# nonl4331/raytracing-rust

Hardware: NVIDIA B200
Metric: Mrays/s (higher is better)
Workload: dtype f32

## Files before the change

### raytracing-rust_b200/csrc/wavefront.cu

```cuda
#include "ptb_internal.h"
#include "ptb_traverse.cuh"
#include "ptb_packet.cuh"
#include "ptb_camcand.cuh"

namespace ptb {

struct RenderParams {
  uint32_t width, height, npix;
  uint32_t row_begin;
  uint32_t tile_w, tile_h;
  uint32_t group;
  uint32_t dir_bins;
  uint32_t sample_offset;
  uint32_t method, max_depth, rr_threshold;
  uint32_t k0, k1;
};

struct Queues {
  uint32_t* live;
  float4* shadow;
  uint32_t* win_count;
  uint32_t* win_prefix;
  uint32_t* seg_total;
  uint8_t* bin;
// ... 204 lines not shown
      uint32_t x, y, sample;
      camera_pixel_sample(rp, first + i, x, y, sample);
      ray = make_ray(sc.cam_origin, camera_direction(sc, rp, x, y, sample));
      return;
    }
    slot = queue[i];
    float4 o, d;
    ldg256_rw(pool.ray + 4u * (size_t)slot, o, d);
    ray = make_ray(from4(o), from4(d));
  }
};
template <bool CAMERA>
struct TraceRetire {
  const PathPool& pool;
  const TraceFetch<CAMERA>& f;
  PTB_DEV void operator()(bool fin, const TraceResult& tr, const Ray& ray) {
    if (fin)
      stg256(pool.ray + 4u * (size_t)f.slot, make_float4(ray.o.x, ray.o.y, ray.o.z, tr.t),
             make_float4(ray.d.x, ray.d.y, ray.d.z, __uint_as_float(tr.ref)));
  }
};

#ifndef PTB_SHADE_MIN_BLOCKS
#define PTB_SHADE_MIN_BLOCKS 4
#endif
template <class TR, bool COUNT, bool CAMERA>
__global__ void __launch_bounds__(256, TR::kTraceMinBlocks)
k_trace(DevScene sc, PathPool pool, Queues q, WaveCounters* wc, RenderParams rp, unsigned long long first) {
  const uint32_t lane = threadIdx.x & 31u;
  uint32_t cnt_nodes = 0, cnt_prims = 0, cnt_rays = 0;
  TraceFetch<CAMERA> fetch{pool, q.live, 0u, sc, rp, first};
  TraceRetire<CAMERA> retire{pool, fetch};
  persistent_trace<TR, false, COUNT>(sc, wc->n_trace, &wc->trace_head, fetch, retire, cnt_nodes, cnt_prims, cnt_rays);
  if (COUNT) {
    for (int off = 16; off > 0; off >>= 1) {
      cnt_nodes += __shfl_xor_sync(0xffffffffu, cnt_nodes, off);
      cnt_prims += __shfl_xor_sync(0xffffffffu, cnt_prims, off);
      cnt_rays += __shfl_xor_sync(0xffffffffu, cnt_rays, off);
    }
    if (lane == 0 && cnt_rays) {
      atomicAdd(&wc->nodes_fetched, (unsigned long long)cnt_nodes);
      atomicAdd(&wc->prims_tested, (unsigned long long)cnt_prims);
      atomicAdd(&wc->rays_counted, (unsigned long long)cnt_rays);
    }
  }
}

#ifndef PTB_CAMERA_MIN_BLOCKS
#define PTB_CAMERA_MIN_BLOCKS 4
#endif
template <bool COUNT>
__global__ void __launch_bounds__(256, PTB_CAMERA_MIN_BLOCKS)
k_trace_camera(DevScene sc, PathPool pool, Queues q, WaveCounters* wc, RenderParams rp, unsigned long long first, CamCandList cl) {
  const uint32_t lane = threadIdx.x & 31u;
  const uint32_t n = wc->n_trace;
  uint32_t cnt_nodes = 0, cnt_prims = 0, cnt_rays = 0;
  for (;;) {
    uint32_t base = 0;
    if (lane == 0u) base = atomicAdd(&wc->trace_head, 32u);
    base = __shfl_sync(0xffffffffu, base, 0);
    if (base >= n) break;
    const uint32_t i = base + lane;
    const bool valid = i < n;
    Ray ray;
    uint32_t lin = 0;
    if (valid) {
      uint32_t x, y, sample;
      camera_pixel_sample(rp, first + i, x, y, sample);
      lin = (y - rp.row_begin) * rp.width + x;
      ray = make_ray(sc.cam_origin, camera_direction(sc, rp, x, y, sample));
      if (COUNT) ++cnt_rays;
    } else {
      ray = make_ray(sc.cam_origin, mk(0.0f, 0.0f, 1.0f));
    }
    float best_t;
    uint32_t best_ref;
    uint32_t cnt = kNone;
    if (cl.count) {
      const uint32_t lin0 = __shfl_sync(0xffffffffu, lin, 0);
      if (__all_sync(0xffffffffu, !valid || lin == lin0)) {
        lin = lin0;
        cnt = __ldg(cl.count + lin);
      }
    }
    if (cnt != kNone) cand_trace<COUNT>(sc, cl, lin, cnt, ray, valid, best_t, best_ref, cnt_prims);
    else packet_trace<COUNT>(sc, ray, valid, best_t, best_ref, cnt_nodes, cnt_prims);
    if (valid)
      stg256(pool.ray + 4u * (size_t)i, make_float4(ray.o.x, ray.o.y, ray.o.z, best_ref == kNone ? 0.0f : best_t),
             make_float4(ray.d.x, ray.d.y, ray.d.z, __uint_as_float(best_ref == kNone ? kNone : (best_ref & ~PTB_LEAF_BIT))));
  }
  if (COUNT) {
    for (int off = 16; off > 0; off >>= 1) {
      cnt_nodes += __shfl_xor_sync(0xffffffffu, cnt_nodes, off);
      cnt_prims += __shfl_xor_sync(0xffffffffu, cnt_prims, off);
      cnt_rays += __shfl_xor_sync(0xffffffffu, cnt_rays, off);
    }
    if (lane == 0 && cnt_rays) {
      atomicAdd(&wc->nodes_fetched, (unsigned long long)cnt_nodes);
      atomicAdd(&wc->prims_tested, (unsigned long long)cnt_prims);
      atomicAdd(&wc->rays_counted, (unsigned long long)cnt_rays);
    }
  }
}

struct Surface {
  HitRec h;
  uint32_t kind, tex, mat;
  float param;
  bool miss;
};

PTB_DEV float tr_d(float alpha, float cos_theta) {
  if (cos_theta <= 0.0f) return 0.0f;
  const float a_sq = alpha * alpha;
  const float tmp = cos_theta * cos_theta * (a_sq - 1.0f) + 1.0f;
  return a_sq / (kPi * tmp * tmp);
}
PTB_DEV float tr_g1(float alpha, v3 normal, v3 h, v3 v) {
  if (dot(v, h) / dot(v, normal) <= 0.0f) return 0.0f;
  const float c = dot(normal, v);
  const float cos_sq = c * c;
  const float alpha_sq = alpha * alpha;
  const float tmp = alpha_sq + (1.0f - alpha_sq) * cos_sq;
// ... 191 lines not shown
        shadow_is_sky = 1u;
      } else {
        const uint32_t lref = __ldg(sc.lights + li);
        l_wi = light_sample_dir(sc, lref, s.h.point, u32_to_unit(r.y), u32_to_unit(r.z));
        const Ray sray = make_ray_from_raw(so, l_wi);
        HitRec si;
        if (prim_hit(sc, sray, lref, si) && si.t > 0.0f) {
          const float pdf = light_pdf(sc, lref, s.h.point, l_wi, si.point, si.normal);
          if (pdf > 0.0f) {
            const uint32_t lmi = __ldg(sc.slot_mat + (lref & kSlotMask)) & 0x00FFFFFFu;
            const DevMaterial* lm = sc.materials + lmi;
            const v3 lpoint = offset_ray(si.point, si.normal, si.error, true);
            le = __ldg(&lm->param) * texture_colour<FULL>(sc, __ldg(&lm->tex), l_wi, lpoint);
            l_pdf = pdf * mult;
            tmax = si.t;
            exclude = lref & kSlotMask;
            usable = true;
          }
        }
      }
      if (usable) {
        const float mp = mat_scattering_pdf<FULL>(s, wo, l_wi);
        const float w = power_heuristic(l_pdf, mp);
        const v3 contrib = T * mat_eval<FULL>(sc, s, wo, l_wi) * w * le / l_pdf;
        const v3 sd = l_wi / mag(l_wi);
        sh_o = make_float4(so.x, so.y, so.z, tmax);
        sh_d = make_float4(sd.x, sd.y, sd.z, __uint_as_float(exclude));
        sh_c = make_float4(contrib.x, contrib.y, contrib.z, __uint_as_float(slot));
        shadow = true;
      }
    }
}

template <int METHOD, bool FULL>
PTB_DEV void shade_path(const DevScene& sc, const PathPool& pool, const RenderParams& rp, uint32_t slot, bool depth0,
                        unsigned long long camera_first, ShadeOut& o) {
  bool &alive = o.alive, &finished = o.finished, &shadow = o.shadow, &contributes = o.contributes;
  uint32_t &shadow_is_sky = o.shadow_is_sky, &fin_pixel = o.fin_pixel;
  float4 &sh_o = o.sh_o, &sh_d = o.sh_d, &sh_c = o.sh_c;
  v3& fin_L = o.fin_L;
  float4 ro, rd, th, ra;
  ldg256_rw(pool.ray + 4u * (size_t)slot, ro, rd);
  if (depth0) {
    uint32_t x, y, smp;
    camera_pixel_sample(rp, camera_first + slot, x, y, smp);
    th = make_float4(1.0f, 1.0f, 1.0f, __uint_as_float(y * rp.width + x));
    ra = make_float4(0.0f, 0.0f, 0.0f, __uint_as_float(smp << 9));
  } else {
    ldg256_rw(pool.col + 4u * (size_t)slot, th, ra);
  }
  const uint2 ht = make_uint2(__float_as_uint(ro.w), __float_as_uint(rd.w));
  const uint32_t pixel = __float_as_uint(th.w);
  const uint32_t df = __float_as_uint(ra.w);
  const uint32_t sample = df >> 9;
  uint32_t depth = df & 0xFFu;
  const bool prev_delta = (df & kFlagPrevDelta) != 0u;
  const Ray ray = make_ray(from4(ro), from4(rd));
  const v3 wo = ray.d;
  v3 T = from4(th), L = from4(ra);

  Surface s;
  s.miss = ht.y == kNone;
  if (s.miss) {
    s.h.t = 0.0f;
    s.h.point = s.h.error = s.h.normal = mk(0.0f, 0.0f, 0.0f);
    s.h.out = false;
    s.kind = PTB_MAT_EMIT;
    s.tex = sc.sky_tex;
    s.mat = 0u;
    s.param = 1.0f;
  } else {
    prim_hit(sc, ray, ht.y, s.h);
    const uint32_t mi = __ldg(sc.slot_mat + (ht.y & kSlotMask)) & 0x00FFFFFFu;
    const DevMaterial* m = sc.materials + mi;
    s.mat = mi;
    s.kind = __ldg(&m->kind);
    s.tex = __ldg(&m->tex);
    s.param = __ldg(&m->param);
  }
  const bool is_emit = s.kind == PTB_MAT_EMIT;
  bool depart = false;
  bool nan_check = true;

  if (METHOD == PTB_METHOD_NAIVE) {
    if (is_emit) {
      const v3 point = offset_ray(s.h.point, s.h.normal, s.h.error, true);
      const v3 emission = s.param * texture_colour<FULL>(sc, s.tex, wo, point);
      L = L + T * emission;
      finished = true;
    } else {
      depart = true;
    }
  } else {
    if (depth == 0u) {
      if (is_emit) {
        const v3 point = offset_ray(s.h.point, s.h.normal, s.h.error, true);
        L = L + s.param * texture_colour<FULL>(sc, s.tex, wo, point);
        finished = true;
        nan_check = false;
      } else {
        depth = 1u;
        depart = true;
      }
    } else {
      if (is_emit) {
        const v3 le = s.param * texture_colour<FULL>(sc, s.tex, wo, ray.o);
        if (!is_zero(le)) {
          const bool sky_samplable = (sc.sky_rx | sc.sky_ry) != 0u;
          const bool use_mis = s.miss ? sky_samplable : !prev_delta;
          if (use_mis) {
            const float divisor = (float)(sky_samplable ? sc.n_lights + 1u : sc.n_lights);
            const float4 pv = pool.prev[slot];
            const float l_pdf = s.miss ? sky_pdf(sc, wo) / divisor
                                       : light_pdf(sc, ht.y, from4(pv), wo, s.h.point, s.h.normal) / divisor;
            const float w = power_heuristic(pv.w, l_pdf);
            L = L + T * le * w;
          } else {
            L = L + T * le;
          }
        }
        finished = true;
      } else {
        bool survive = true;
        if (depth > rp.rr_threshold) {
          const float p = cmax3(T.x, T.y, T.z);
          const uint4 r = philox4x32_10(pixel, sample, (depth << 8) | RNG_RR, 0u, rp.k0, rp.k1);
          if (u32_to_unit(r.x) > p) survive = false;
          else T = T / p;
        }
        depth += 1u;
        if (survive && depth < rp.max_depth) depart = true;
        else finished = true;
      }
    }
  }

  if (depart) {
    float m_pdf = 0.0f;
    if (METHOD == PTB_METHOD_MIS) nee_sample<FULL>(sc, rp, s, wo, T, pixel, sample, depth, slot, o);
    const uint4 r = philox4x32_10(pixel, sample, (depth << 8) | RNG_SCATTER, 0u, rp.k0, rp.k1);
    v3 new_o, new_dir;
    bool delta = false;
    if (s.kind == PTB_MAT_LAMBERTIAN) {
      new_dir = lambertian_sample_dir(s.h.normal, u32_to_unit(r.x), u32_to_unit(r.y));
      new_o = offset_ray(s.h.point, s.h.normal, s.h.error, true);
    } else if (FULL && s.kind == PTB_MAT_TROWBRIDGE_REITZ) {
      new_dir = tr_sample(s.param, -wo, s.h.normal, u32_to_unit(r.x), u32_to_unit(r.y));
// ... 37 lines not shown
        else T = T / p;
      }
      depth += 1u;
      if (survive && depth < rp.max_depth) alive = true;
      else finished = true;
    } else {
      if (s.kind == PTB_MAT_LAMBERTIAN) {
        m_pdf = fmaxf(dot(nd, s.h.normal), 0.0f) / kPi;
        T = T * (col * s.param);
      } else if (is_tr) {
        m_pdf = mat_scattering_pdf<FULL>(s, wo, nd);
        T = T * col;
      } else {
        m_pdf = 0.0f;
        T = T * (col / 0.0f);
      }
      pool.prev[slot] = make_float4(s.h.point.x, s.h.point.y, s.h.point.z, m_pdf);
      alive = true;
    }
    if (alive) {
      stg256(pool.ray + 4u * (size_t)slot, make_float4(new_o.x, new_o.y, new_o.z, 0.0f),
             make_float4(nd.x, nd.y, nd.z, __uint_as_float(kNone)));
      stg256(pool.col + 4u * (size_t)slot, make_float4(T.x, T.y, T.z, th.w),
             make_float4(L.x, L.y, L.z, __uint_as_float((sample << 9) | (delta ? kFlagPrevDelta : 0u) | depth)));
      o.bin = rp.dir_bins ? direction_bin(nd) : 0u;
    }
  }
  if (finished) {
    contributes = !(nan_check && (contains_nan(L) || !any_finite(L)));
    fin_pixel = pixel;
    fin_L = L;
  }
}

template <int METHOD, bool FULL>
__global__ void __launch_bounds__(256, PTB_SHADE_MIN_BLOCKS + (METHOD == PTB_METHOD_MIS ? 1 : 0))
k_shade(DevScene sc, PathPool pool, Queues q, WaveCounters* wc, RenderParams rp, float* __restrict__ accum,
        unsigned long long camera_first, uint32_t sort_kinds) {
  const bool depth0 = camera_first != kNoCamera;
  const uint32_t lane = threadIdx.x & 31u;
  const uint32_t n_total = wc->n_trace;
  for (uint32_t base = blockIdx.x * blockDim.x; base < n_total; base += gridDim.x * blockDim.x) {
  const uint32_t i = base + threadIdx.x;
  bool active = i < n_total;

  uint32_t slot = 0;
  ShadeOut so;
  so.fin_L = mk(0.0f, 0.0f, 0.0f);

  if (active) slot = depth0 ? i : q.live[i];
  if (sort_kinds) {
    __shared__ uint32_t s_slot[256];
    __shared__ uint32_t s_cnt[(kNumKinds + 1) * 8];
    const uint32_t warp = threadIdx.x >> 5, n_warps = blockDim.x >> 5;
    uint32_t kind = (uint32_t)kNumKinds;
    if (active) {
      const uint32_t ref = __float_as_uint(pool.ray[4u * (size_t)slot + 1u].w);
      kind = ref == kNone ? 0u : 1u + (__ldg(sc.slot_mat + (ref & kSlotMask)) >> 24);
    }
    uint32_t rank = 0;
#pragma unroll
    for (uint32_t k = 0; k <= (uint32_t)kNumKinds; ++k) {
      const uint32_t m = __ballot_sync(0xffffffffu, kind == k);
      if (kind == k) rank = (uint32_t)__popc(m & ((1u << lane) - 1u));
      if (lane == 0u) s_cnt[k * 8u + warp] = (uint32_t)__popc(m);
    }
    __syncthreads();
    uint32_t pos = rank;
    for (uint32_t e = 0; e < kind * 8u + warp; ++e)
      if ((e & 7u) < n_warps) pos += s_cnt[e];
    s_slot[pos] = slot;
    __syncthreads();
    uint32_t n_here = 0;
    for (uint32_t e = 0; e < (uint32_t)kNumKinds * 8u; ++e)
      if ((e & 7u) < n_warps) n_here += s_cnt[e];
    active = threadIdx.x < n_here;
    slot = s_slot[threadIdx.x];
    __syncthreads();
  }
  if (active) shade_path<METHOD, FULL>(sc, pool, rp, slot, depth0, camera_first, so);
  finish_paths(accum, so.contributes, so.fin_pixel, so.fin_L);

  if (so.alive) q.bin[slot] = (uint8_t)so.bin;
  if (so.finished) q.bin[slot] = (uint8_t)kBinDead;
  const uint32_t window = slot / kWindow;
  const uint32_t peers = __match_any_sync(0xffffffffu, so.finished ? window : 0xffffffffu);
  if (so.finished && lane == (uint32_t)__ffs(peers) - 1u) atomicSub(&q.win_count[window], (uint32_t)__popc(peers));
  if (METHOD == PTB_METHOD_MIS) {
    const uint32_t m_sh = __ballot_sync(0xffffffffu, so.shadow), m_sky = __ballot_sync(0xffffffffu, so.shadow && so.shadow_is_sky);
    unsigned long long p2 = 0ull;
    if (lane == 0u && m_sh)
      p2 = atomicAdd(&wc->shadow_pair, ((unsigned long long)__popc(m_sky) << 32) | (unsigned long long)__popc(m_sh));
    p2 = __shfl_sync(0xffffffffu, p2, 0);
    if (so.shadow) {
      float4* e = q.shadow + 3u * (size_t)((uint32_t)p2 + __popc(m_sh & ((1u << lane) - 1u)));
      e[0] = so.sh_o;
      e[1] = so.sh_d;
      e[2] = so.sh_c;
    }
  }
  }
}

__global__ void __launch_bounds__(256) k_win_init(Queues q, WaveCounters* wc, uint32_t n_paths) {
  const uint32_t w = blockIdx.x * blockDim.x + threadIdx.x;
  if (w == 0u) {
    wc->mode = 0u; wc->n_tail = 0u; wc->tail_iter = 0xFFFFFFFFu; wc->n_trace = 0u; wc->tail_head = 0u;
    if (wc->tail_t0 != ~0ull && wc->tail_t1 > wc->tail_t0) wc->tail_ns += wc->tail_t1 - wc->tail_t0;
    wc->tail_t0 = ~0ull;
    wc->tail_t1 = 0ull;
  }
  if (w < q.n_windows) {
    const unsigned long long first = (unsigned long long)w * kWindow;
    q.win_count[w] = first >= n_paths ? 0u : (n_paths - first < kWindow ? (uint32_t)(n_paths - first) : kWindow);
  }
}

__global__ void __launch_bounds__(1024) k_win_scan(Queues q) {
  __shared__ uint32_t warp_sum[32];
  const uint32_t lane = threadIdx.x & 31u, warp = threadIdx.x >> 5;
  const uint32_t w0 = blockIdx.x * kSegWindows + threadIdx.x * 4u;
  uint32_t c[4];
#pragma unroll
  for (int k = 0; k < 4; ++k) c[k] = w0 + k < q.n_windows ? q.win_count[w0 + k] : 0u;
  const uint32_t mine = c[0] + c[1] + c[2] + c[3];
  uint32_t inc = mine;
#pragma unroll
  for (int o = 1; o < 32; o <<= 1) {
    const uint32_t t = __shfl_up_sync(0xffffffffu, inc, o);
    if (lane >= (uint32_t)o) inc += t;
  }
  if (lane == 31u) warp_sum[warp] = inc;
  __syncthreads();
// ... 151 lines not shown
  }
};
struct ShadowRetire {
  const PathPool& pool;
  const ShadowFetch& f;
  PTB_DEV void operator()(bool fin, const TraceResult& tr, const Ray&) {
    if (fin && tr.ref == kNone) {
      const uint32_t slot = __float_as_uint(f.contrib.w);
      float4 ra = pool.col[4u * (size_t)slot + 1u];
      ra.x += f.contrib.x; ra.y += f.contrib.y; ra.z += f.contrib.z;
      pool.col[4u * (size_t)slot + 1u] = ra;
    }
  }
};
#ifndef PTB_SHADOW_MIN_BLOCKS
#define PTB_SHADOW_MIN_BLOCKS 1
#endif
template <class TR>
__global__ void __launch_bounds__(256, PTB_SHADOW_MIN_BLOCKS) k_shadow(DevScene sc, PathPool pool, Queues q, WaveCounters* wc) {
  uint32_t a = 0, b = 0, r = 0;
  ShadowFetch fetch{q, make_float4(0.f, 0.f, 0.f, 0.f)};
  ShadowRetire retire{pool, fetch};
  persistent_trace<TR, true, false>(sc, (uint32_t)wc->shadow_pair, &wc->shadow_head, fetch, retire, a, b, r);
}

PTB_DEV unsigned long long global_timer_ns() {
  unsigned long long t;
  asm volatile("mov.u64 %0, %%globaltimer;" : "=l"(t));
  return t;
}
template <int METHOD, bool FULL>
PTB_DEV void tail_shade(const DevScene& sc, const PathPool& pool, const RenderParams& rp, uint32_t slot, const Ray& ray,
                        const TraceResult& tr, ShadeOut& so) {
  stg256(pool.ray + 4u * (size_t)slot, make_float4(ray.o.x, ray.o.y, ray.o.z, tr.t),
         make_float4(ray.d.x, ray.d.y, ray.d.z, __uint_as_float(tr.ref)));
  so.fin_L = mk(0.0f, 0.0f, 0.0f);
  shade_path<METHOD, FULL>(sc, pool, rp, slot, false, kNoCamera, so);
}
PTB_DEV void tail_add_nee(const PathPool& pool, uint32_t slot, const ShadeOut& so) {
  float4 ra = pool.col[4u * (size_t)slot + 1u];
  ra.x += so.sh_c.x; ra.y += so.sh_c.y; ra.z += so.sh_c.z;
  pool.col[4u * (size_t)slot + 1u] = ra;
}
PTB_DEV void tail_finish(float* __restrict__ accum, const Queues& q, uint32_t slot, const ShadeOut& so) {
  if (so.contributes) {
    atomicAdd(accum + 3u * (size_t)so.fin_pixel + 0, so.fin_L.x);
    atomicAdd(accum + 3u * (size_t)so.fin_pixel + 1, so.fin_L.y);
    atomicAdd(accum + 3u * (size_t)so.fin_pixel + 2, so.fin_L.z);
  }
  q.bin[slot] = (uint8_t)kBinDead;
}

constexpr uint32_t kCoopMinPrims = 4096u;
#ifndef PTB_TAIL_WARPS
#define PTB_TAIL_WARPS 4
#endif
constexpr int kTailThreads = 32 * PTB_TAIL_WARPS;
template <class TR, int METHOD, bool FULL>
__global__ void __launch_bounds__(kTailThreads)
k_tail(DevScene sc, PathPool pool, Queues q, WaveCounters* wc, RenderParams rp, float* __restrict__ accum, uint32_t depth) {
  if (wc->tail_iter != depth) return;
  const uint32_t n = wc->n_tail;
  if (threadIdx.x == 0u) atomicMin(&wc->tail_t0, global_timer_ns());
#ifdef PTB_TAIL_STATS
  if (threadIdx.x == 0u) atomicMin(&g_tail_stats[9], global_timer_ns());
#endif
  constexpr bool COOP = TR::kCoop;
  __shared__ CoopWarp s_coop[COOP ? PTB_TAIL_WARPS : 1];
  const uint32_t lane = threadIdx.x & 31u, warp = threadIdx.x >> 5;
  unsigned long long c_bounce = 0, c_sky = 0, c_light = 0, c_ref = 0, c_paths = 0;
// ... 401 lines not shown
  return PTB_OK;
}

template <class TR>
static const void* trace_kernel_of(bool count, bool camera) {
  if (camera) return count ? (const void*)k_trace<TR, true, true> : (const void*)k_trace<TR, false, true>;
  return count ? (const void*)k_trace<TR, true, false> : (const void*)k_trace<TR, false, false>;
}
static const void* trace_kernel(const Ctx* c, bool count, bool camera) {
  return c->wide ? trace_kernel_of<CwTrav>(count, camera) : trace_kernel_of<BinTrav>(count, camera);
}
static const void* shadow_kernel(const Ctx* c) { return c->wide ? (const void*)k_shadow<CwTrav> : (const void*)k_shadow<BinTrav>; }
static const void* api_kernel(const Ctx* c, bool count) {
  if (c->wide) return count ? (const void*)k_closest_hit_api<CwTrav, true> : (const void*)k_closest_hit_api<CwTrav, false>;
  return count ? (const void*)k_closest_hit_api<BinTrav, true> : (const void*)k_closest_hit_api<BinTrav, false>;
}
static const void* aov_kernel(const Ctx* c) { return c->wide ? (const void*)k_aov<CwTrav> : (const void*)k_aov<BinTrav>; }
static const void* visibility_kernel(const Ctx* c, bool chi) {
  if (c->wide) return chi ? (const void*)k_visibility_api<CwTrav, true> : (const void*)k_visibility_api<CwTrav, false>;
  return chi ? (const void*)k_visibility_api<BinTrav, true> : (const void*)k_visibility_api<BinTrav, false>;
}
template <class TR>
static const void* tail_kernel_of(bool mis, bool full) {
  if (mis) return full ? (const void*)k_tail<TR, PTB_METHOD_MIS, true> : (const void*)k_tail<TR, PTB_METHOD_MIS, false>;
  return full ? (const void*)k_tail<TR, PTB_METHOD_NAIVE, true> : (const void*)k_tail<TR, PTB_METHOD_NAIVE, false>;
}
static cudaError_t launch_trace(const void* fn, int grid, cudaStream_t st, const DevScene& sc, const PathPool& pool, const Queues& q,
                                WaveCounters* wc, const RenderParams& rp, unsigned long long first) {
  void* args[] = {(void*)&sc, (void*)&pool, (void*)&q, (void*)&wc, (void*)&rp, (void*)&first};
  return cudaLaunchKernel(fn, dim3((unsigned)grid), dim3(256), args, 0, st);
}
static cudaError_t launch_trace_camera(const void* fn, int grid, cudaStream_t st, const DevScene& sc, const PathPool& pool,
                                       const Queues& q, WaveCounters* wc, const RenderParams& rp, unsigned long long first,
                                       const CamCandList& cl) {
  void* args[] = {(void*)&sc, (void*)&pool, (void*)&q, (void*)&wc, (void*)&rp, (void*)&first, (void*)&cl};
  return cudaLaunchKernel(fn, dim3((unsigned)grid), dim3(256), args, 0, st);
}
static cudaError_t launch_shadow(const void* fn, int grid, cudaStream_t st, const DevScene& sc, const PathPool& pool, const Queues& q,
                                 WaveCounters* wc) {
  void* args[] = {(void*)&sc, (void*)&pool, (void*)&q, (void*)&wc};
  return cudaLaunchKernel(fn, dim3((unsigned)grid), dim3(256), args, 0, st);
}

static int persistent_grid(Ctx* c, const void* kernel, int threads) {
  int per_sm = 0;
  if (cudaOccupancyMaxActiveBlocksPerMultiprocessor(&per_sm, kernel, threads, 0) != cudaSuccess || per_sm < 1) per_sm = 1;
  return c->sm_count * per_sm;
}

static int32_t prepare_batch(Ctx* c, const float4* r4, size_t n, uint32_t** head, unsigned long long** counts,
                             const uint32_t** order) {
  if (n > 0xFFFFFFF0ull) return set_error(c, PTB_ERR_INVALID, "too many rays in one batch");
  PTB_CUDA_TRY(c, c->d_counters.reserve(sizeof(WaveCounters) + 64));
  char* scratch = c->d_counters.as<char>() + sizeof(WaveCounters);
  *head = reinterpret_cast<uint32_t*>(scratch);
  *counts = reinterpret_cast<unsigned long long*>(scratch + 8);
  PTB_CUDA_TRY(c, cudaMemsetAsync(scratch, 0, 24, c->stream));
  *order = nullptr;
  bool sort = n >= (1u << 16) && c->n_prims > 0;
  if (const char* e = getenv("PTB_HIT_SORT")) sort = sort && atoi(e) != 0;
  if (sort) {
    const uint32_t n32 = (uint32_t)n;
    PTB_CUDA_TRY(c, c->d_hit_sort.reserve(((size_t)n32 * 4 + radix_sort_hist_words(n32)) * 4));
    uint32_t* w = c->d_hit_sort.as<uint32_t>();
    uint32_t *ka = w, *va = w + n, *kb = w + 2 * n, *vb = w + 3 * n, *hist = w + 4 * n;
    k_ray_sort_keys<<<(n32 + 255u) / 256u, 256, 0, c->stream>>>(c->dev, r4, n32, ka, va);
    c->stats.kernel_launches += 1;
    radix_sort_pairs(c, ka, va, kb, vb, n32, 3, hist);
// ... 314 lines not shown
  c->stats.paths += h.paths;
  c->stats.wavefront_iterations += iterations;
}
struct SlotRefs {
  const PathPool& pool;
  const Queues& q;
  WaveCounters* wc;
};
static void launch_shade(const RenderSetup& rs, Ctx* c, const SlotRefs& sl, uint32_t grid, int threads, cudaStream_t st,
                         unsigned long long camera_first) {
  const uint32_t sort = rs.sort_kinds ? 1u : 0u;
  if (rs.mis) {
    if (rs.full) k_shade<PTB_METHOD_MIS, true><<<grid, threads, 0, st>>>(c->dev, sl.pool, sl.q, sl.wc, rs.rp, rs.accum, camera_first, sort);
    else k_shade<PTB_METHOD_MIS, false><<<grid, threads, 0, st>>>(c->dev, sl.pool, sl.q, sl.wc, rs.rp, rs.accum, camera_first, sort);
  } else {
    if (rs.full) k_shade<PTB_METHOD_NAIVE, true><<<grid, threads, 0, st>>>(c->dev, sl.pool, sl.q, sl.wc, rs.rp, rs.accum, camera_first, sort);
    else k_shade<PTB_METHOD_NAIVE, false><<<grid, threads, 0, st>>>(c->dev, sl.pool, sl.q, sl.wc, rs.rp, rs.accum, camera_first, sort);
  }
}
static const void* tail_fn(const RenderSetup& rs, Ctx* c) {
  return c->wide ? tail_kernel_of<CwTrav>(rs.mis, rs.full) : tail_kernel_of<BinTrav>(rs.mis, rs.full);
}
static void launch_tail(const RenderSetup& rs, Ctx* c, const SlotRefs& sl, uint32_t grid, cudaStream_t st, uint32_t depth) {
  const void* fn = tail_fn(rs, c);
  WaveCounters* wc = sl.wc;
  float* accum = rs.accum;
  void* args[] = {(void*)&c->dev, (void*)&sl.pool, (void*)&sl.q, (void*)&wc, (void*)&rs.rp, (void*)&accum, (void*)&depth};
  cudaLaunchKernel(fn, dim3(grid), dim3(kTailThreads), args, 0, st);
}
static const void* shade_fn(const RenderSetup& rs) {
  return rs.mis ? (rs.full ? (const void*)k_shade<PTB_METHOD_MIS, true> : (const void*)k_shade<PTB_METHOD_MIS, false>)
                : (rs.full ? (const void*)k_shade<PTB_METHOD_NAIVE, true> : (const void*)k_shade<PTB_METHOD_NAIVE, false>);
}

static int32_t render_window_mode(Ctx* c, const ptb_render_opts& o, const RenderSetup& rs, ptb_progress_fn progress, void* user) {
  cudaStream_t st = c->stream;
  const uint32_t npix = rs.rp.npix, P = rs.chunk_paths;
  const unsigned long long total = (unsigned long long)npix * o.samples_per_pixel;
  const bool mis = rs.mis, prof = rs.prof, count = rs.count;
  const int T = 256;
  const SlotRefs slots[2] = {{c->pool, rs.q, rs.wc}, {rs.pool2, rs.q2, rs.wc2}};
  const uint32_t n_windows = rs.q.n_windows;
  const uint32_t n_seg = (n_windows + kSegWindows - 1) / kSegWindows;
  auto capped = [&](const void* k, uint32_t items_per_block, uint32_t items) {
    const uint32_t g = (uint32_t)persistent_grid(c, k, T), need = (items + items_per_block - 1) / items_per_block;
    return g < need ? g : (need ? need : 1u);
  };
  const uint32_t grid_fill = capped((const void*)k_win_fill, kFillGroup, n_windows);
  int TS = 128;
  if (const char* e = getenv("PTB_SHADE_THREADS")) { int v = atoi(e); if (v == 64 || v == 128 || v == 256) TS = v; }
  uint32_t grid_shade = (uint32_t)persistent_grid(c, shade_fn(rs), TS);
  if (grid_shade > (P + TS - 1) / TS) grid_shade = (P + TS - 1) / TS;
  const void* fn_trace = trace_kernel(c, count, false);
  bool cam_packet = !c->wide && rs.rp.group % 32u == 0u;
  if (const char* e = getenv("PTB_CAMERA_PACKET")) cam_packet = !c->wide && atoi(e) != 0;
  const void* fn_trace_cam = cam_packet ? (count ? (const void*)k_trace_camera<true> : (const void*)k_trace_camera<false>)
                                        : trace_kernel(c, count, true);
  const bool cand_ok = cam_packet && rs.rp.group % 32u == 0u;
  bool cam_cand = cand_ok && c->n_prims >= 4096;
  if (const char* e = getenv("PTB_CAMERA_CAND")) cam_cand = cand_ok && atoi(e) != 0;
  CamCandList cand{nullptr, nullptr, kCamCandMaxK};
  if (const char* e = getenv("PTB_CAMERA_CAND_K")) { int v = atoi(e); if (v >= 1 && v <= (int)kCamCandMaxK) cand.k = (uint32_t)v; }
  if (cam_cand) {
    PTB_CUDA_TRY(c, c->d_camcand.reserve((size_t)npix * cand.k * sizeof(uint4)));
    PTB_CUDA_TRY(c, c->d_camcand_count.reserve((size_t)npix * sizeof(uint32_t)));
    cand.entries = c->d_camcand.as<uint4>();
    cand.count = c->d_camcand_count.as<uint32_t>();
  }
  const void* fn_shadow = shadow_kernel(c);
  const int grid_trace = persistent_grid(c, fn_trace, T);
  const int grid_trace_cam = persistent_grid(c, fn_trace_cam, T);
  const int grid_shadow = persistent_grid(c, fn_shadow, T);
  int cam_fetch = c->dev.trace_fetch_threshold < 4 ? c->dev.trace_fetch_threshold : 4;
  if (const char* e = getenv("PTB_TRACE_FETCH_CAMERA")) { int v = atoi(e); if (v >= 1 && v <= 32) cam_fetch = v; }
  uint32_t tail_paths = 65536u;
  if (const char* e = getenv("PTB_TAIL_PATHS")) { long v = atol(e); if (v >= 0 && v <= (1l << 24)) tail_paths = (uint32_t)v; }
  if (count) tail_paths = 0u;
  if (tail_paths) {
    if (!c->s_tail) {
      int lo = 0, hi = 0;
      cudaDeviceGetStreamPriorityRange(&lo, &hi);
      PTB_CUDA_TRY(c, cudaStreamCreateWithPriority(&c->s_tail, cudaStreamNonBlocking, hi));
    }
    for (int k = 0; k < 2; ++k) {
      if (!c->ev_head_done[k]) PTB_CUDA_TRY(c, cudaEventCreateWithFlags(&c->ev_head_done[k], cudaEventDisableTiming));
      if (!c->ev_tail_done[k]) PTB_CUDA_TRY(c, cudaEventCreateWithFlags(&c->ev_tail_done[k], cudaEventDisableTiming));
    }
  }
  for (cudaEvent_t& e : c->ev_ring)
    if (!e) PTB_CUDA_TRY(c, cudaEventCreateWithFlags(&e, cudaEventDisableTiming));
// ... 74 lines not shown
      PTB_CUDA_TRY(c, cudaStreamWaitEvent(s, c->ev_tail_done[sl], 0));
    PTB_CUDA_TRY(c, cudaMemsetAsync(S.q.win_count, 0, (size_t)S.q.n_windows * 4, s));
    if (R.n_paths % kWindow)
      PTB_CUDA_TRY(c, cudaMemsetAsync(S.q.bin + R.n_paths, (int)kBinDead, kWindow - R.n_paths % kWindow, s));
    prof_rec(sl, 0, 0, 0);
    k_win_init<<<(S.q.n_windows + T - 1) / T, T, 0, s>>>(S.q, S.wc, R.n_paths);
    c->stats.kernel_launches += 1;
    return PTB_OK;
  };
  auto enqueue_iteration = [&](int sl) -> int32_t {
    ChunkRun& R = run[sl];
    const SlotRefs& S = slots[sl];
    const Queues& q = S.q;
    WaveCounters* wc = S.wc;
    cudaStream_t s = wst[sl];
    const uint64_t depth = R.depth;
    if (depth) prof_rec(sl, depth, 0, 0);
    k_win_scan<<<n_seg, 1024, 0, s>>>(q);
    k_win_prepare<<<1, 32, 0, s>>>(wc, q, n_seg, o.method, depth == 0 ? 0u : (depth == 1 ? 1u : 2u), (uint32_t)depth, tail_paths);
    if (depth) k_win_fill<<<grid_fill, T, 0, s>>>(q, wc);
    prof_rec(sl, depth, 0, 1);
    if (tail_paths && depth >= 2) {
      PTB_CUDA_TRY(c, cudaEventRecord(c->ev_head_done[sl], s));
      PTB_CUDA_TRY(c, cudaStreamWaitEvent(c->s_tail, c->ev_head_done[sl], 0));
      launch_tail(rs, c, S, R.last ? grid_tail_last : grid_tail, c->s_tail, (uint32_t)depth);
      PTB_CUDA_TRY(c, cudaEventRecord(c->ev_tail_done[sl], c->s_tail));
      R.tail_pending = true;
      c->stats.kernel_launches += 1;
    }
    prof_rec(sl, depth, 1, 0);
    if (depth == 0) {
      DevScene cam = c->dev;
      cam.trace_fetch_threshold = cam_fetch;
      if (cam_packet) PTB_CUDA_TRY(c, launch_trace_camera(fn_trace_cam, grid_trace_cam, s, cam, S.pool, q, wc, rs.rp, R.first, cand));
      else PTB_CUDA_TRY(c, launch_trace(fn_trace_cam, grid_trace_cam, s, cam, S.pool, q, wc, rs.rp, R.first));
    } else {
      PTB_CUDA_TRY(c, launch_trace(fn_trace, grid_trace, s, c->dev, S.pool, q, wc, rs.rp, 0ull));
    }
    prof_rec(sl, depth, 1, 1);
    prof_rec(sl, depth, 2, 0);
    launch_shade(rs, c, S, grid_shade, TS, s, depth == 0 ? R.first : kNoCamera);
    prof_rec(sl, depth, 2, 1);
    c->stats.kernel_launches += depth ? 5 : 4;
    c->stats.trace_launches += 1;
    if (mis) {
      prof_rec(sl, depth, 3, 0);
      PTB_CUDA_TRY(c, launch_shadow(fn_shadow, grid_shadow, s, c->dev, S.pool, q, wc));
      prof_rec(sl, depth, 3, 1);
      c->stats.kernel_launches += 1;
    }
    const int r = sl * 4 + (int)(depth & 3u);
    PTB_CUDA_TRY(c, cudaMemcpyAsync(c->h_counters + r, wc, sizeof(WaveCounters), cudaMemcpyDeviceToHost, s));
    PTB_CUDA_TRY(c, cudaEventRecord(c->ev_ring[r], s));
    ++R.depth;
    ++iterations;
    if (R.depth > 4096) return set_error(c, PTB_ERR_INVALID, "wavefront did not terminate");
    return PTB_OK;
  };
  auto drain_one = [&](int sl) {
    ChunkRun& R = run[sl];
    const int r = sl * 4 + (int)(R.drained & 3u);
    if (prof) prof_collect(c, r, mis);
    if (c->h_counters[r].mode != 0u) R.over = true;
    R.rays_ref_seen = c->h_counters[r].rays_reference;
    ++R.drained;
  };

  while (rc == PTB_OK) {
    while (next_first < total && (int)run[0].active + (int)run[1].active < chunk_streams) {
      const int sl = two ? (int)(chunks_started & 1u) : 0;
      if (run[sl].active) break;
      const int32_t e = start_chunk(sl);
      if (e != PTB_OK) return e;
    }
    if (!run[0].active && !run[1].active) break;
    bool progress_made = false;
// ... 62 lines not shown
```

Before: 5493.

## Fuse camera-ray shading into packet camera trace kernel, skip depth-0 shade launch

The packet camera trace kernel now shades its hit in place, calling a new shade_hit helper and routing results (bins, shadow rays, accumulation) itself, so the separate depth-0 shade launch is dropped. This avoids writing camera rays and hits to the pool and reading them back, and saves one kernel launch per chunk. The tail shade path likewise passes the ray and hit directly instead of storing them and reloading. In exchange the fused kernel carries both trace and shade register pressure at the camera min-blocks bound, and it loses the shade kernel's kind sorting for depth-0 paths.

```diff
diff --git a/raytracing-rust_b200/csrc/wavefront.cu b/raytracing-rust_b200/csrc/wavefront.cu
--- a/raytracing-rust_b200/csrc/wavefront.cu
+++ b/raytracing-rust_b200/csrc/wavefront.cu
@@ -260,63 +260,6 @@
   TraceFetch<CAMERA> fetch{pool, q.live, 0u, sc, rp, first};
   TraceRetire<CAMERA> retire{pool, fetch};
   persistent_trace<TR, false, COUNT>(sc, wc->n_trace, &wc->trace_head, fetch, retire, cnt_nodes, cnt_prims, cnt_rays);
-  if (COUNT) {
-    for (int off = 16; off > 0; off >>= 1) {
-      cnt_nodes += __shfl_xor_sync(0xffffffffu, cnt_nodes, off);
-      cnt_prims += __shfl_xor_sync(0xffffffffu, cnt_prims, off);
-      cnt_rays += __shfl_xor_sync(0xffffffffu, cnt_rays, off);
-    }
-    if (lane == 0 && cnt_rays) {
-      atomicAdd(&wc->nodes_fetched, (unsigned long long)cnt_nodes);
-      atomicAdd(&wc->prims_tested, (unsigned long long)cnt_prims);
-      atomicAdd(&wc->rays_counted, (unsigned long long)cnt_rays);
-    }
-  }
-}
-
-#ifndef PTB_CAMERA_MIN_BLOCKS
-#define PTB_CAMERA_MIN_BLOCKS 4
-#endif
-template <bool COUNT>
-__global__ void __launch_bounds__(256, PTB_CAMERA_MIN_BLOCKS)
-k_trace_camera(DevScene sc, PathPool pool, Queues q, WaveCounters* wc, RenderParams rp, unsigned long long first, CamCandList cl) {
-  const uint32_t lane = threadIdx.x & 31u;
-  const uint32_t n = wc->n_trace;
-  uint32_t cnt_nodes = 0, cnt_prims = 0, cnt_rays = 0;
-  for (;;) {
-    uint32_t base = 0;
-    if (lane == 0u) base = atomicAdd(&wc->trace_head, 32u);
-    base = __shfl_sync(0xffffffffu, base, 0);
-    if (base >= n) break;
-    const uint32_t i = base + lane;
-    const bool valid = i < n;
-    Ray ray;
-    uint32_t lin = 0;
-    if (valid) {
-      uint32_t x, y, sample;
-      camera_pixel_sample(rp, first + i, x, y, sample);
-      lin = (y - rp.row_begin) * rp.width + x;
-      ray = make_ray(sc.cam_origin, camera_direction(sc, rp, x, y, sample));
-      if (COUNT) ++cnt_rays;
-    } else {
-      ray = make_ray(sc.cam_origin, mk(0.0f, 0.0f, 1.0f));
-    }
-    float best_t;
-    uint32_t best_ref;
-    uint32_t cnt = kNone;
-    if (cl.count) {
-      const uint32_t lin0 = __shfl_sync(0xffffffffu, lin, 0);
-      if (__all_sync(0xffffffffu, !valid || lin == lin0)) {
-        lin = lin0;
-        cnt = __ldg(cl.count + lin);
-      }
-    }
-    if (cnt != kNone) cand_trace<COUNT>(sc, cl, lin, cnt, ray, valid, best_t, best_ref, cnt_prims);
-    else packet_trace<COUNT>(sc, ray, valid, best_t, best_ref, cnt_nodes, cnt_prims);
-    if (valid)
-      stg256(pool.ray + 4u * (size_t)i, make_float4(ray.o.x, ray.o.y, ray.o.z, best_ref == kNone ? 0.0f : best_t),
-             make_float4(ray.d.x, ray.d.y, ray.d.z, __uint_as_float(best_ref == kNone ? kNone : (best_ref & ~PTB_LEAF_BIT))));
-  }
   if (COUNT) {
     for (int off = 16; off > 0; off >>= 1) {
       cnt_nodes += __shfl_xor_sync(0xffffffffu, cnt_nodes, off);
@@ -574,35 +517,27 @@
     }
 }
 
+PTB_DEV void camera_colour(uint32_t pixel, uint32_t sample, float4& th, float4& ra) {
+  th = make_float4(1.0f, 1.0f, 1.0f, __uint_as_float(pixel));
+  ra = make_float4(0.0f, 0.0f, 0.0f, __uint_as_float(sample << 9));
+}
 template <int METHOD, bool FULL>
-PTB_DEV void shade_path(const DevScene& sc, const PathPool& pool, const RenderParams& rp, uint32_t slot, bool depth0,
-                        unsigned long long camera_first, ShadeOut& o) {
+PTB_DEV void shade_hit(const DevScene& sc, const PathPool& pool, const RenderParams& rp, uint32_t slot, const Ray& ray,
+                       uint32_t hit_ref, float4 th, float4 ra, ShadeOut& o) {
   bool &alive = o.alive, &finished = o.finished, &shadow = o.shadow, &contributes = o.contributes;
   uint32_t &shadow_is_sky = o.shadow_is_sky, &fin_pixel = o.fin_pixel;
   float4 &sh_o = o.sh_o, &sh_d = o.sh_d, &sh_c = o.sh_c;
   v3& fin_L = o.fin_L;
-  float4 ro, rd, th, ra;
-  ldg256_rw(pool.ray + 4u * (size_t)slot, ro, rd);
-  if (depth0) {
-    uint32_t x, y, smp;
-    camera_pixel_sample(rp, camera_first + slot, x, y, smp);
-    th = make_float4(1.0f, 1.0f, 1.0f, __uint_as_float(y * rp.width + x));
-    ra = make_float4(0.0f, 0.0f, 0.0f, __uint_as_float(smp << 9));
-  } else {
-    ldg256_rw(pool.col + 4u * (size_t)slot, th, ra);
-  }
-  const uint2 ht = make_uint2(__float_as_uint(ro.w), __float_as_uint(rd.w));
   const uint32_t pixel = __float_as_uint(th.w);
   const uint32_t df = __float_as_uint(ra.w);
   const uint32_t sample = df >> 9;
   uint32_t depth = df & 0xFFu;
   const bool prev_delta = (df & kFlagPrevDelta) != 0u;
-  const Ray ray = make_ray(from4(ro), from4(rd));
   const v3 wo = ray.d;
   v3 T = from4(th), L = from4(ra);
 
   Surface s;
-  s.miss = ht.y == kNone;
+  s.miss = hit_ref == kNone;
   if (s.miss) {
     s.h.t = 0.0f;
     s.h.point = s.h.error = s.h.normal = mk(0.0f, 0.0f, 0.0f);
@@ -612,8 +547,8 @@
     s.mat = 0u;
     s.param = 1.0f;
   } else {
-    prim_hit(sc, ray, ht.y, s.h);
-    const uint32_t mi = __ldg(sc.slot_mat + (ht.y & kSlotMask)) & 0x00FFFFFFu;
+    prim_hit(sc, ray, hit_ref, s.h);
+    const uint32_t mi = __ldg(sc.slot_mat + (hit_ref & kSlotMask)) & 0x00FFFFFFu;
     const DevMaterial* m = sc.materials + mi;
     s.mat = mi;
     s.kind = __ldg(&m->kind);
@@ -654,7 +589,7 @@
             const float divisor = (float)(sky_samplable ? sc.n_lights + 1u : sc.n_lights);
             const float4 pv = pool.prev[slot];
             const float l_pdf = s.miss ? sky_pdf(sc, wo) / divisor
-                                       : light_pdf(sc, ht.y, from4(pv), wo, s.h.point, s.h.normal) / divisor;
+                                       : light_pdf(sc, hit_ref, from4(pv), wo, s.h.point, s.h.normal) / divisor;
             const float w = power_heuristic(pv.w, l_pdf);
             L = L + T * le * w;
           } else {
@@ -758,55 +693,25 @@
     fin_L = L;
   }
 }
-
 template <int METHOD, bool FULL>
-__global__ void __launch_bounds__(256, PTB_SHADE_MIN_BLOCKS + (METHOD == PTB_METHOD_MIS ? 1 : 0))
-k_shade(DevScene sc, PathPool pool, Queues q, WaveCounters* wc, RenderParams rp, float* __restrict__ accum,
-        unsigned long long camera_first, uint32_t sort_kinds) {
-  const bool depth0 = camera_first != kNoCamera;
+PTB_DEV void shade_path(const DevScene& sc, const PathPool& pool, const RenderParams& rp, uint32_t slot, bool depth0,
+                        unsigned long long camera_first, ShadeOut& o) {
+  float4 ro, rd, th, ra;
+  ldg256_rw(pool.ray + 4u * (size_t)slot, ro, rd);
+  if (depth0) {
+    uint32_t x, y, smp;
+    camera_pixel_sample(rp, camera_first + slot, x, y, smp);
+    camera_colour(y * rp.width + x, smp, th, ra);
+  } else {
+    ldg256_rw(pool.col + 4u * (size_t)slot, th, ra);
+  }
+  shade_hit<METHOD, FULL>(sc, pool, rp, slot, make_ray(from4(ro), from4(rd)), __float_as_uint(rd.w), th, ra, o);
+}
+
+template <int METHOD>
+PTB_DEV void route_shaded(float* __restrict__ accum, const Queues& q, WaveCounters* wc, uint32_t slot, const ShadeOut& so) {
   const uint32_t lane = threadIdx.x & 31u;
-  const uint32_t n_total = wc->n_trace;
-  for (uint32_t base = blockIdx.x * blockDim.x; base < n_total; base += gridDim.x * blockDim.x) {
-  const uint32_t i = base + threadIdx.x;
-  bool active = i < n_total;
-
-  uint32_t slot = 0;
-  ShadeOut so;
-  so.fin_L = mk(0.0f, 0.0f, 0.0f);
-
-  if (active) slot = depth0 ? i : q.live[i];
-  if (sort_kinds) {
-    __shared__ uint32_t s_slot[256];
-    __shared__ uint32_t s_cnt[(kNumKinds + 1) * 8];
-    const uint32_t warp = threadIdx.x >> 5, n_warps = blockDim.x >> 5;
-    uint32_t kind = (uint32_t)kNumKinds;
-    if (active) {
-      const uint32_t ref = __float_as_uint(pool.ray[4u * (size_t)slot + 1u].w);
-      kind = ref == kNone ? 0u : 1u + (__ldg(sc.slot_mat + (ref & kSlotMask)) >> 24);
-    }
-    uint32_t rank = 0;
-#pragma unroll
-    for (uint32_t k = 0; k <= (uint32_t)kNumKinds; ++k) {
-      const uint32_t m = __ballot_sync(0xffffffffu, kind == k);
-      if (kind == k) rank = (uint32_t)__popc(m & ((1u << lane) - 1u));
-      if (lane == 0u) s_cnt[k * 8u + warp] = (uint32_t)__popc(m);
-    }
-    __syncthreads();
-    uint32_t pos = rank;
-    for (uint32_t e = 0; e < kind * 8u + warp; ++e)
-      if ((e & 7u) < n_warps) pos += s_cnt[e];
-    s_slot[pos] = slot;
-    __syncthreads();
-    uint32_t n_here = 0;
-    for (uint32_t e = 0; e < (uint32_t)kNumKinds * 8u; ++e)
-      if ((e & 7u) < n_warps) n_here += s_cnt[e];
-    active = threadIdx.x < n_here;
-    slot = s_slot[threadIdx.x];
-    __syncthreads();
-  }
-  if (active) shade_path<METHOD, FULL>(sc, pool, rp, slot, depth0, camera_first, so);
   finish_paths(accum, so.contributes, so.fin_pixel, so.fin_L);
-
   if (so.alive) q.bin[slot] = (uint8_t)so.bin;
   if (so.finished) q.bin[slot] = (uint8_t)kBinDead;
   const uint32_t window = slot / kWindow;
@@ -825,6 +730,118 @@
       e[2] = so.sh_c;
     }
   }
+}
+
+template <int METHOD, bool FULL>
+__global__ void __launch_bounds__(256, PTB_SHADE_MIN_BLOCKS + (METHOD == PTB_METHOD_MIS ? 1 : 0))
+k_shade(DevScene sc, PathPool pool, Queues q, WaveCounters* wc, RenderParams rp, float* __restrict__ accum,
+        unsigned long long camera_first, uint32_t sort_kinds) {
+  const bool depth0 = camera_first != kNoCamera;
+  const uint32_t lane = threadIdx.x & 31u;
+  const uint32_t n_total = wc->n_trace;
+  for (uint32_t base = blockIdx.x * blockDim.x; base < n_total; base += gridDim.x * blockDim.x) {
+  const uint32_t i = base + threadIdx.x;
+  bool active = i < n_total;
+
+  uint32_t slot = 0;
+  ShadeOut so;
+  so.fin_L = mk(0.0f, 0.0f, 0.0f);
+
+  if (active) slot = depth0 ? i : q.live[i];
+  if (sort_kinds) {
+    __shared__ uint32_t s_slot[256];
+    __shared__ uint32_t s_cnt[(kNumKinds + 1) * 8];
+    const uint32_t warp = threadIdx.x >> 5, n_warps = blockDim.x >> 5;
+    uint32_t kind = (uint32_t)kNumKinds;
+    if (active) {
+      const uint32_t ref = __float_as_uint(pool.ray[4u * (size_t)slot + 1u].w);
+      kind = ref == kNone ? 0u : 1u + (__ldg(sc.slot_mat + (ref & kSlotMask)) >> 24);
+    }
+    uint32_t rank = 0;
+#pragma unroll
+    for (uint32_t k = 0; k <= (uint32_t)kNumKinds; ++k) {
+      const uint32_t m = __ballot_sync(0xffffffffu, kind == k);
+      if (kind == k) rank = (uint32_t)__popc(m & ((1u << lane) - 1u));
+      if (lane == 0u) s_cnt[k * 8u + warp] = (uint32_t)__popc(m);
+    }
+    __syncthreads();
+    uint32_t pos = rank;
+    for (uint32_t e = 0; e < kind * 8u + warp; ++e)
+      if ((e & 7u) < n_warps) pos += s_cnt[e];
+    s_slot[pos] = slot;
+    __syncthreads();
+    uint32_t n_here = 0;
+    for (uint32_t e = 0; e < (uint32_t)kNumKinds * 8u; ++e)
+      if ((e & 7u) < n_warps) n_here += s_cnt[e];
+    active = threadIdx.x < n_here;
+    slot = s_slot[threadIdx.x];
+    __syncthreads();
+  }
+  if (active) shade_path<METHOD, FULL>(sc, pool, rp, slot, depth0, camera_first, so);
+  route_shaded<METHOD>(accum, q, wc, slot, so);
+  }
+}
+
+#ifndef PTB_CAMERA_MIN_BLOCKS
+#define PTB_CAMERA_MIN_BLOCKS 4
+#endif
+template <int METHOD, bool FULL, bool COUNT>
+__global__ void __launch_bounds__(256, PTB_CAMERA_MIN_BLOCKS)
+k_trace_camera(DevScene sc, PathPool pool, Queues q, WaveCounters* wc, RenderParams rp, unsigned long long first, CamCandList cl,
+               float* __restrict__ accum) {
+  const uint32_t lane = threadIdx.x & 31u;
+  const uint32_t n = wc->n_trace;
+  uint32_t cnt_nodes = 0, cnt_prims = 0, cnt_rays = 0;
+  for (;;) {
+    uint32_t base = 0;
+    if (lane == 0u) base = atomicAdd(&wc->trace_head, 32u);
+    base = __shfl_sync(0xffffffffu, base, 0);
+    if (base >= n) break;
+    const uint32_t i = base + lane;
+    const bool valid = i < n;
+    Ray ray;
+    uint32_t lin = 0, sample = 0;
+    if (valid) {
+      uint32_t x, y;
+      camera_pixel_sample(rp, first + i, x, y, sample);
+      lin = (y - rp.row_begin) * rp.width + x;
+      ray = make_ray(sc.cam_origin, camera_direction(sc, rp, x, y, sample));
+      if (COUNT) ++cnt_rays;
+    } else {
+      ray = make_ray(sc.cam_origin, mk(0.0f, 0.0f, 1.0f));
+    }
+    float best_t;
+    uint32_t best_ref;
+    uint32_t cnt = kNone;
+    if (cl.count) {
+      const uint32_t lin0 = __shfl_sync(0xffffffffu, lin, 0);
+      if (__all_sync(0xffffffffu, !valid || lin == lin0)) {
+        lin = lin0;
+        cnt = __ldg(cl.count + lin);
+      }
+    }
+    if (cnt != kNone) cand_trace<COUNT>(sc, cl, lin, cnt, ray, valid, best_t, best_ref, cnt_prims);
+    else packet_trace<COUNT>(sc, ray, valid, best_t, best_ref, cnt_nodes, cnt_prims);
+    ShadeOut so;
+    so.fin_L = mk(0.0f, 0.0f, 0.0f);
+    if (valid) {
+      float4 th, ra;
+      camera_colour(lin + rp.row_begin * rp.width, sample, th, ra);
+      shade_hit<METHOD, FULL>(sc, pool, rp, i, ray, best_ref == kNone ? kNone : (best_ref & ~PTB_LEAF_BIT), th, ra, so);
+    }
+    route_shaded<METHOD>(accum, q, wc, i, so);
+  }
+  if (COUNT) {
+    for (int off = 16; off > 0; off >>= 1) {
+      cnt_nodes += __shfl_xor_sync(0xffffffffu, cnt_nodes, off);
+      cnt_prims += __shfl_xor_sync(0xffffffffu, cnt_prims, off);
+      cnt_rays += __shfl_xor_sync(0xffffffffu, cnt_rays, off);
+    }
+    if (lane == 0 && cnt_rays) {
+      atomicAdd(&wc->nodes_fetched, (unsigned long long)cnt_nodes);
+      atomicAdd(&wc->prims_tested, (unsigned long long)cnt_prims);
+      atomicAdd(&wc->rays_counted, (unsigned long long)cnt_rays);
+    }
   }
 }
 
@@ -1042,10 +1059,10 @@
 template <int METHOD, bool FULL>
 PTB_DEV void tail_shade(const DevScene& sc, const PathPool& pool, const RenderParams& rp, uint32_t slot, const Ray& ray,
                         const TraceResult& tr, ShadeOut& so) {
-  stg256(pool.ray + 4u * (size_t)slot, make_float4(ray.o.x, ray.o.y, ray.o.z, tr.t),
-         make_float4(ray.d.x, ray.d.y, ray.d.z, __uint_as_float(tr.ref)));
+  float4 th, ra;
+  ldg256_rw(pool.col + 4u * (size_t)slot, th, ra);
   so.fin_L = mk(0.0f, 0.0f, 0.0f);
-  shade_path<METHOD, FULL>(sc, pool, rp, slot, false, kNoCamera, so);
+  shade_hit<METHOD, FULL>(sc, pool, rp, slot, ray, tr.ref, th, ra, so);
 }
 PTB_DEV void tail_add_nee(const PathPool& pool, uint32_t slot, const ShadeOut& so) {
   float4 ra = pool.col[4u * (size_t)slot + 1u];
@@ -1513,8 +1530,8 @@
 }
 static cudaError_t launch_trace_camera(const void* fn, int grid, cudaStream_t st, const DevScene& sc, const PathPool& pool,
                                        const Queues& q, WaveCounters* wc, const RenderParams& rp, unsigned long long first,
-                                       const CamCandList& cl) {
-  void* args[] = {(void*)&sc, (void*)&pool, (void*)&q, (void*)&wc, (void*)&rp, (void*)&first, (void*)&cl};
+                                       const CamCandList& cl, float* accum) {
+  void* args[] = {(void*)&sc, (void*)&pool, (void*)&q, (void*)&wc, (void*)&rp, (void*)&first, (void*)&cl, (void*)&accum};
   return cudaLaunchKernel(fn, dim3((unsigned)grid), dim3(256), args, 0, st);
 }
 static cudaError_t launch_shadow(const void* fn, int grid, cudaStream_t st, const DevScene& sc, const PathPool& pool, const Queues& q,
@@ -1895,6 +1912,14 @@
   return rs.mis ? (rs.full ? (const void*)k_shade<PTB_METHOD_MIS, true> : (const void*)k_shade<PTB_METHOD_MIS, false>)
                 : (rs.full ? (const void*)k_shade<PTB_METHOD_NAIVE, true> : (const void*)k_shade<PTB_METHOD_NAIVE, false>);
 }
+template <int METHOD>
+static const void* trace_camera_of(bool full, bool count) {
+  if (full) return count ? (const void*)k_trace_camera<METHOD, true, true> : (const void*)k_trace_camera<METHOD, true, false>;
+  return count ? (const void*)k_trace_camera<METHOD, false, true> : (const void*)k_trace_camera<METHOD, false, false>;
+}
+static const void* trace_camera_fn(const RenderSetup& rs) {
+  return rs.mis ? trace_camera_of<PTB_METHOD_MIS>(rs.full, rs.count) : trace_camera_of<PTB_METHOD_NAIVE>(rs.full, rs.count);
+}
 
 static int32_t render_window_mode(Ctx* c, const ptb_render_opts& o, const RenderSetup& rs, ptb_progress_fn progress, void* user) {
   cudaStream_t st = c->stream;
@@ -1917,8 +1942,7 @@
   const void* fn_trace = trace_kernel(c, count, false);
   bool cam_packet = !c->wide && rs.rp.group % 32u == 0u;
   if (const char* e = getenv("PTB_CAMERA_PACKET")) cam_packet = !c->wide && atoi(e) != 0;
-  const void* fn_trace_cam = cam_packet ? (count ? (const void*)k_trace_camera<true> : (const void*)k_trace_camera<false>)
-                                        : trace_kernel(c, count, true);
+  const void* fn_trace_cam = cam_packet ? trace_camera_fn(rs) : trace_kernel(c, count, true);
   const bool cand_ok = cam_packet && rs.rp.group % 32u == 0u;
   bool cam_cand = cand_ok && c->n_prims >= 4096;
   if (const char* e = getenv("PTB_CAMERA_CAND")) cam_cand = cand_ok && atoi(e) != 0;
@@ -2059,16 +2083,17 @@
     if (depth == 0) {
       DevScene cam = c->dev;
       cam.trace_fetch_threshold = cam_fetch;
-      if (cam_packet) PTB_CUDA_TRY(c, launch_trace_camera(fn_trace_cam, grid_trace_cam, s, cam, S.pool, q, wc, rs.rp, R.first, cand));
+      if (cam_packet) PTB_CUDA_TRY(c, launch_trace_camera(fn_trace_cam, grid_trace_cam, s, cam, S.pool, q, wc, rs.rp, R.first, cand, rs.accum));
       else PTB_CUDA_TRY(c, launch_trace(fn_trace_cam, grid_trace_cam, s, cam, S.pool, q, wc, rs.rp, R.first));
     } else {
       PTB_CUDA_TRY(c, launch_trace(fn_trace, grid_trace, s, c->dev, S.pool, q, wc, rs.rp, 0ull));
     }
     prof_rec(sl, depth, 1, 1);
+    const bool shade = depth || !cam_packet;
     prof_rec(sl, depth, 2, 0);
-    launch_shade(rs, c, S, grid_shade, TS, s, depth == 0 ? R.first : kNoCamera);
+    if (shade) launch_shade(rs, c, S, grid_shade, TS, s, depth == 0 ? R.first : kNoCamera);
     prof_rec(sl, depth, 2, 1);
-    c->stats.kernel_launches += depth ? 5 : 4;
+    c->stats.kernel_launches += (depth ? 4 : 3) + (shade ? 1 : 0);
     c->stats.trace_launches += 1;
     if (mis) {
       prof_rec(sl, depth, 3, 0);
```

Result: faster. 5590, median of 6 (+1.8%).
